# nanoporetech/medaka

Hardware: NVIDIA H100
Metric: pileup positions/sec (consensus inference) (higher is better)
Workload: dtype f32

## Files before the change

### include/medaka_b200.h

```cpp
#ifndef MEDAKA_B200_H
#define MEDAKA_B200_H

#include <stddef.h>
#include <stdint.h>

#ifdef __cplusplus
extern "C" {
#endif

#define MDK_OK 0
#define MDK_ERR_ARG -1
#define MDK_ERR_CUDA -2
#define MDK_ERR_STATE -3
#define MDK_ERR_UNSUPPORTED -4
#define MDK_ERR_NOMEM -5

#define MDK_PREC_TC 0
#define MDK_PREC_FP32 1

#define MDK_REC_AUTO 0
#define MDK_REC_ONE_TILE 1
#define MDK_REC_PINGPONG 2

#define MDK_NORM_TOTAL 0
// ... 184 lines not shown
                            float *ref_q_out, int64_t *n_runs_out, int64_t *n_run_cols_out);

int mdk_variant_columns(int device, const int64_t *minor, const uint8_t *reference,
                        const uint8_t *prediction, uint8_t *out, int64_t len);

int mdk_decode_variants(int device, const float *probs, const int64_t *minor, const uint8_t *ref_code, int64_t n,
                        uint8_t *pred_out, uint8_t *is_var_out, float *pred_q_out, float *ref_q_out, int64_t max_runs,
                        int64_t *run_start, int64_t *run_len, float *run_pred_q, float *run_ref_q,
                        int64_t *n_runs_out);

int mdk_selftest_umma(int device, const float *A, const float *B, float *D, int N, int K,
                      int variant);

int mdk_debug_timeline(mdk_engine *e, int n_last, float *out);
int mdk_debug_read_plog(mdk_engine *e, float *out_host, int64_t n_floats);
int mdk_rl_debug_read(mdk_rl_engine *e, int which, float *out_host, int64_t n_floats);

typedef struct mdk_trainer mdk_trainer;

#define MDK_OPT_RMSPROP 0
#define MDK_OPT_ADAM 1
#define MDK_OPT_NADAM 2
#define MDK_OPT_SGD 3

typedef struct mdk_optim_desc {
    int32_t kind;
    float alpha, beta1, beta2, eps, weight_decay, momentum, dampening, momentum_decay;
    int32_t nesterov;
} mdk_optim_desc;

// ... 49 lines not shown
```

### medaka_b200/csrc/api.cu

```cuda
#include <algorithm>
#include <cstdlib>
#include <cstring>
#include <new>

#include "common.cuh"
#include "gru_pack.cuh"

namespace mdk {

static thread_local std::string g_last_error;

void set_error(const std::string &msg) { g_last_error = msg; }

int cuda_fail(cudaError_t err, const char *what, const char *file, int line) {
    char buf[512];
    snprintf(buf, sizeof(buf), "CUDA error %d (%s) at %s:%d: %s", (int)err, cudaGetErrorString(err), file, line, what);
    g_last_error = buf;
    if (err == cudaErrorMemoryAllocation) {
        cudaGetLastError();
        return MDK_ERR_NOMEM;
    }
    return MDK_ERR_CUDA;
}

// ... 136 lines not shown
}

static int ensure_var(mdk_lane &ln) {
    if (ln.cap_var >= ln.cap_io && ln.d_ref) return MDK_OK;
    dev_free(ln.d_ref); dev_free(ln.d_calls); dev_free(ln.d_pred_q); dev_free(ln.d_ref_q);
    ln.cap_var = 0;
    int rc;
    if ((rc = dev_alloc(&ln.d_ref, (size_t)ln.cap_io))) return rc;
    if ((rc = dev_alloc(&ln.d_calls, (size_t)ln.cap_io))) return rc;
    if ((rc = dev_alloc(&ln.d_pred_q, (size_t)ln.cap_io))) return rc;
    if ((rc = dev_alloc(&ln.d_ref_q, (size_t)ln.cap_io))) return rc;
    ln.cap_var = ln.cap_io;
    return MDK_OK;
}

static int run_forward256(mdk_engine *e, mdk_ws &ws, const float *feats_dev, int64_t B, int64_t T, float *probs_dev,
                          float *logits_dev, uint8_t *labels_dev, uint8_t *quals_dev, const HeadVariant *var) {
    int rc;
    if ((rc = ensure_h1(ws, H2_256))) return rc;
    const int64_t P = B * T;
    cudaStream_t s = ws.stream, s1 = ws.l1_stream;
    const bool tc = e->precision == MDK_PREC_TC;
    const LayerWeights &l0 = e->layer[0], &l1 = e->layer[1];
    float *h0 = static_cast<float *>(ws.h0);
    MDK_CUDA(cudaStreamWaitEvent(s, ws.l1_done, 0));
    MDK_CUDA(cudaEventRecord(e->ev[1], s));
    MDK_CUDA(launch_inproj0(feats_dev, l0.w_in_packed, l0.bias_gi, ws.gi, P, e->desc.num_features,
                            T, tc ? 1 : 0, s, H256));
    MDK_CUDA(cudaEventRecord(e->ev[2], s));
    if (tc) MDK_CUDA(launch_rec256_tc(ws.gi, l0.w_hh_tm, l0.b_hn_tc, h0, B, T, s));
    else MDK_CUDA(launch_rec_fp32(ws.gi, l0.w_hh_t, l0.b_hn, h0, B, T, s, H256));
    MDK_CUDA(cudaEventRecord(e->ev[3], s));
    if (tc) MDK_CUDA(launch_gemm256_tc(h0, l1.w_in_tc, l1.bias_gi_tc, ws.gi, tiled_rows(B, T), s));
    else MDK_CUDA(launch_gemm_fp32(h0, l1.w_in_packed, l1.bias_gi, ws.gi, P, H2_256, GI256_COLS, s));
    MDK_CUDA(cudaEventRecord(e->ev[4], s));
    MDK_CUDA(cudaStreamWaitEvent(s1, e->ev[4], 0));
    if (tc) MDK_CUDA(launch_rec256_tc(ws.gi, l1.w_hh_tm, l1.b_hn_tc, ws.h1, B, T, s1));
    else MDK_CUDA(launch_rec_fp32(ws.gi, l1.w_hh_t, l1.b_hn, ws.h1, B, T, s1, H256));
    MDK_CUDA(cudaEventRecord(e->ev[5], s1));
    MDK_CUDA(cudaEventRecord(ws.l1_done, s1));
    MDK_CUDA(launch_head(ws.h1, e->lin_w, e->lin_b, B, T, tc ? 1 : 0, probs_dev, logits_dev, labels_dev, s1, quals_dev,
                         var, H2_256));
    MDK_CUDA(cudaEventRecord(e->ev[6], s1));
    e->launches += 5;
    e->last.launches = 5;
    ws.last_fused_head = false;
    ws.last_B = B; ws.last_T = T; ws.last_precision = e->precision;
    e->last_ws = (int)(&ws - e->ws);
    return MDK_OK;
}

static int run_forward(mdk_engine *e, mdk_ws &ws, const float *feats_dev, int64_t B, int64_t T, float *probs_dev,
                       float *logits_dev, uint8_t *labels_dev, uint8_t *quals_dev, const HeadVariant *var) {
    int rc;
    if ((rc = prepare_weights(e))) return rc;
    if ((rc = ensure_workspace(e, ws, B, T))) return rc;
    if (e->desc.gru_size == H256)
        return run_forward256(e, ws, feats_dev, B, T, probs_dev, logits_dev, labels_dev, quals_dev, var);
    const int64_t P = B * T;
    cudaStream_t s = ws.stream, s1 = ws.l1_stream;
    const bool tc = e->precision == MDK_PREC_TC;
    int launches = 0;
    const bool fuse_x = tc && e->layer[0].w_x_tm != nullptr;
    const int64_t tiles = (B + WT - 1) / WT;
    const int tiles_per_cta = e->rec_mode == MDK_REC_PINGPONG ? 2
                            : e->rec_mode == MDK_REC_ONE_TILE ? 1
                            : fuse_x || tiles * NDIR > (int64_t)e->sm_count ? 2 : 1;
    const bool fuse_head = tc && !e->keep_act;
    if (!fuse_head && (rc = ensure_h1(ws, H2))) return rc;
    if (!fuse_x) MDK_CUDA(cudaStreamWaitEvent(s, ws.l1_done, 0));
    MDK_CUDA(cudaEventRecord(e->ev[1], s));
    if (!fuse_x) {
        MDK_CUDA(launch_inproj0(feats_dev, e->layer[0].w_in_packed, e->layer[0].bias_gi, ws.gi, P,
                                e->desc.num_features, T, tc ? 1 : 0, s));
        launches++;
    }
    MDK_CUDA(cudaEventRecord(e->ev[2], s));
    if (tc) {
        const RecX fx{feats_dev, e->layer[0].w_x_tm, e->layer[0].bias_gi_tc, e->desc.num_features};
        MDK_CUDA(launch_rec_tc(ws.gi, fuse_x ? &fx : nullptr, e->layer[0].w_hh_tm, e->layer[0].b_hn_tc, tiles_per_cta,
                               OUT_TILES, ws.h0, nullptr, B, T, s));
    } else {
        MDK_CUDA(launch_rec_fp32(ws.gi, e->layer[0].w_hh_t, e->layer[0].b_hn, (float *)ws.h0, B, T, s));
    }
    launches++;
    if (fuse_x) MDK_CUDA(cudaStreamWaitEvent(s, ws.l1_done, 0));
    MDK_CUDA(cudaEventRecord(e->ev[3], s));
    if (tc) MDK_CUDA(launch_gemm_tc(ws.h0, e->layer[1].w_in_tc, e->layer[1].bias_gi_tc, ws.gi, tiled_rows(B, T), e->sm_count, s));
    else MDK_CUDA(launch_gemm_fp32((const float *)ws.h0, e->layer[1].w_in_packed, e->layer[1].bias_gi, ws.gi, P, H2, GI_COLS, s));
    launches++;
    MDK_CUDA(cudaEventRecord(e->ev[4], s));
    MDK_CUDA(cudaStreamWaitEvent(s1, e->ev[4], 0));
    if (tc) {
        MDK_CUDA(launch_rec_tc(ws.gi, nullptr, e->layer[1].w_hh_tm, e->layer[1].b_hn_tc, tiles_per_cta,
                               fuse_head ? OUT_LOGITS : OUT_ROWS, fuse_head ? (void *)ws.plog : ws.h1, e->lin_w, B, T, s1));
    } else {
        MDK_CUDA(launch_rec_fp32(ws.gi, e->layer[1].w_hh_t, e->layer[1].b_hn, ws.h1, B, T, s1));
    }
    launches++;
    MDK_CUDA(cudaEventRecord(e->ev[5], s1));
    MDK_CUDA(cudaEventRecord(ws.l1_done, s1));
    if (fuse_head) MDK_CUDA(launch_head_plog(ws.plog, e->lin_b, B, T, probs_dev, logits_dev, labels_dev, s1, quals_dev, var));
    else MDK_CUDA(launch_head(ws.h1, e->lin_w, e->lin_b, B, T, tc ? 1 : 0, probs_dev, logits_dev, labels_dev, s1, quals_dev,
                              var));
    launches++;
    MDK_CUDA(cudaEventRecord(e->ev[6], s1));
    e->launches += launches;
    e->last.launches = launches;
    ws.last_fused_head = fuse_head;
    ws.last_B = B; ws.last_T = T; ws.last_precision = e->precision;
    e->last_ws = (int)(&ws - e->ws);
    return MDK_OK;
}

static int acquire_lane(mdk_engine *e, int64_t P, int *out) {
    int idx;
    if (P > mdk_engine::SMALL_POS) {
        idx = e->next_big;
        e->next_big = (e->next_big + 1) % mdk_engine::BIG_LANES;
    } else {
        idx = mdk_engine::BIG_LANES + e->next_small;
        e->next_small = (e->next_small + 1) % mdk_engine::SMALL_LANES;
    }
    mdk_lane &ln = e->lane[idx];
    if (ln.busy) {
        MDK_CUDA(cudaEventSynchronize(ln.ev_out));
        ln.busy = false;
    }
    *out = idx;
    return MDK_OK;
}

struct GruCall {
    mdk_engine *e;
    const float *feats = nullptr;
    int64_t B = 0, T = 0;
    const uint8_t *ref = nullptr;

    int open(int64_t windows) {
        const int rc = acquire_lane(e, B * T, &e->open_lane);
        return rc ? rc : ensure_io(e, e->lane[e->open_lane], windows, T);
    }
    int64_t capacity(int64_t len) {
        const mdk_lane &ln = e->lane[e->open_lane];
        return std::min(ln.cap_io / len, ln.cap_feats / (len * e->desc.num_features));
    }
    int stage(int64_t first, int64_t n, int64_t at) {
        const size_t w = (size_t)T * e->desc.num_features;
        mdk_lane &ln = e->lane[e->open_lane];
        MDK_CUDA(cudaMemcpyAsync(ln.d_feats + at * w, feats + first * w, n * w * sizeof(float), cudaMemcpyDefault,
                                 e->copy_in));
        if (ref) {
            int rc;
            if ((rc = ensure_var(ln))) return rc;
            MDK_CUDA(cudaMemcpyAsync(ln.d_ref + at * T, ref + first * T, n * T, cudaMemcpyDefault, e->copy_in));
        }
        return MDK_OK;
    }
    int launch() {
        mdk_lane &ln = e->lane[e->open_lane];
        const Packing &pk = e->pk;
        bool logits = false, labels = false, quals = false, var = false;
        for (const Packing::Piece &p : pk.pieces) {
            logits = logits || p.logits; labels = labels || (p.labels && !p.ref); quals = quals || p.quals;
            var = var || p.ref;
        }
        const HeadVariant hv{ln.d_ref, ln.d_calls, ln.d_pred_q, ln.d_ref_q};
        int rc;
        if (quals && (rc = ensure_quals(ln))) return rc;
        cudaStream_t s = ln.ws->stream;
        e->ev = e->evr[e->fwd_count % mdk_engine::EV_RING];
        e->fwd_count++;
        MDK_CUDA(cudaEventRecord(e->ev[0], s));
        MDK_CUDA(cudaEventRecord(ln.ev_in, e->copy_in));
        MDK_CUDA(cudaStreamWaitEvent(s, ln.ev_in, 0));
        if ((rc = run_forward(e, *ln.ws, ln.d_feats, pk.windows, pk.len, ln.d_probs, logits ? ln.d_logits : nullptr,
                              labels ? ln.d_labels : nullptr, quals ? ln.d_quals : nullptr, var ? &hv : nullptr)))
            return rc;
        MDK_CUDA(cudaEventRecord(e->ev[7], ln.ws->l1_stream));
        if ((rc = copy_back(e->copy_out, pk, ln.ws->l1_stream, ln.d_probs, ln.d_logits, ln.d_labels, ln.d_quals, &hv)))
            return rc;
        MDK_CUDA(cudaEventRecord(ln.ev_out, e->copy_out.stream));
        ln.busy = true;
        return MDK_OK;
    }
};

static int launch_group(mdk_engine *e) { return e->pk.launch(GruCall{e}); }

static int64_t group_limit(mdk_engine *e) {
    return e->group_windows > 0 ? e->group_windows : mdk_engine_preferred_windows(e);
}

static float ev_ms(cudaEvent_t a, cudaEvent_t b) {
    float ms = 0.f;
    if (cudaEventElapsedTime(&ms, a, b) != cudaSuccess) { cudaGetLastError(); return -1.f; }
    return ms;
}

static int check_shapes(const mdk_engine *e, const void *feats, int64_t B, int64_t T, const void *probs) {
    MDK_REQUIRE(e != nullptr, MDK_ERR_ARG, "engine is NULL");
    MDK_REQUIRE(feats != nullptr && probs != nullptr, MDK_ERR_ARG, "forward: feats/probs must not be NULL");
    MDK_REQUIRE(B >= 1 && T >= 1, MDK_ERR_ARG, "forward: need B >= 1 and T >= 1");
// ... 118 lines not shown
    }
    e->stream = e->ws[0].stream;
    for (auto &set : e->evr) for (auto &ev : set) cudaEventCreate(&ev);
    cudaStreamCreateWithFlags(&e->copy_in, cudaStreamNonBlocking);
    for (auto &ev : e->ev_timer) cudaEventCreate(&ev);
    cudaEventCreateWithFlags(&e->ev_join, cudaEventDisableTiming);
    cudaError_t err = create_copy_out(e->copy_out);
    if (err != cudaSuccess) { mdk_engine_destroy(e); return cuda_fail(err, "create_copy_out", __FILE__, __LINE__); }
    *out = e;
    return MDK_OK;
}

int mdk_engine_destroy(mdk_engine *e) {
    if (!e) return MDK_OK;
    cudaSetDevice(e->device);
    for (auto &ws : e->ws) {
        if (ws.stream) cudaStreamSynchronize(ws.stream);
        if (ws.l1_stream) cudaStreamSynchronize(ws.l1_stream);
    }
    destroy_copy_out(e->copy_out);
    for (auto &ws : e->ws) {
        dev_free(ws.gi); dev_free(ws.h1); dev_free(ws.plog);
        if (ws.h0) cudaFree(ws.h0);
        if (ws.stream) cudaStreamDestroy(ws.stream);
        if (ws.l1_stream) cudaStreamDestroy(ws.l1_stream);
        if (ws.l1_done) cudaEventDestroy(ws.l1_done);
    }
    for (auto &ln : e->lane) {
        dev_free(ln.d_feats); dev_free(ln.d_probs); dev_free(ln.d_logits); dev_free(ln.d_labels); dev_free(ln.d_quals);
        dev_free(ln.d_ref); dev_free(ln.d_calls); dev_free(ln.d_pred_q); dev_free(ln.d_ref_q);
        if (ln.ev_in) cudaEventDestroy(ln.ev_in);
        if (ln.ev_out) cudaEventDestroy(ln.ev_out);
    }
    if (e->copy_in) cudaStreamDestroy(e->copy_in);
    for (auto &set : e->evr) for (auto &ev : set) if (ev) cudaEventDestroy(ev);
    for (auto &ev : e->ev_timer) if (ev) cudaEventDestroy(ev);
    if (e->ev_join) cudaEventDestroy(e->ev_join);
    delete e;
    cudaGetLastError();
    return MDK_OK;
}

static int quiesce(mdk_engine *e) {
    int rc = launch_group(e);
    if (rc) return rc;
    for (auto &ws : e->ws) MDK_CUDA(ws_sync(ws));
    return MDK_OK;
}

int mdk_engine_load_gru(mdk_engine *e, int layer, int direction, const float *w_ih, const float *w_hh,
                        const float *b_ih, const float *b_hh) {
    MDK_REQUIRE(e, MDK_ERR_ARG, "engine is NULL");
    MDK_REQUIRE(layer >= 0 && layer < 2 && direction >= 0 && direction < 2, MDK_ERR_ARG, "load_gru: bad layer/direction");
    MDK_REQUIRE(w_ih && w_hh && b_ih && b_hh, MDK_ERR_ARG, "load_gru: NULL weight pointer");
    MDK_CUDA(cudaSetDevice(e->device));
    { int rcq = quiesce(e); if (rcq) return rcq; }
    LayerWeights &lw = e->layer[layer];
    const int g3 = 3 * e->desc.gru_size;
    lw.w_ih[direction].assign(w_ih, w_ih + (size_t)g3 * in_features(e, layer));
// ... 34 lines not shown
                "set_rec_mode: at gru_size 256 the recurrence has one kernel; only MDK_REC_AUTO applies");
    e->rec_mode = mode;
    return MDK_OK;
}

int mdk_engine_set_group_windows(mdk_engine *e, int64_t windows) {
    MDK_REQUIRE(e && windows >= 0, MDK_ERR_ARG, "set_group_windows: bad arguments");
    e->group_windows = windows;
    return MDK_OK;
}

int mdk_engine_reserve(mdk_engine *e, int64_t B, int64_t T) {
    MDK_REQUIRE(e && B >= 1 && T >= 1, MDK_ERR_ARG, "reserve: bad arguments");
    MDK_CUDA(cudaSetDevice(e->device));
    int rc;
    if ((rc = launch_group(e))) return rc;
    if (e->desc.gru_size == H256) B = std::min(B, group_limit(e));
    const bool big = B * T > mdk_engine::SMALL_POS;
    const int l0 = big ? 0 : mdk_engine::BIG_LANES, l1 = big ? mdk_engine::BIG_LANES : mdk_engine::N_LANES;
    for (int i = l0; i < l1; ++i) {
        mdk_lane &ln = e->lane[i];
        if (ln.busy) { MDK_CUDA(cudaEventSynchronize(ln.ev_out)); ln.busy = false; }
        if ((rc = ensure_workspace(e, *ln.ws, B, T))) return rc;
        if ((rc = ensure_io(e, ln, B, T))) return rc;
    }
    return MDK_OK;
}

int mdk_engine_forward_dev(mdk_engine *e, const float *feats_dev, int64_t B, int64_t T, float *probs_dev,
                           float *logits_dev, uint8_t *labels_dev) {
    int rc;
// ... 32 lines not shown
    MDK_REQUIRE(e != nullptr, MDK_ERR_ARG, "engine is NULL");
    MDK_REQUIRE(feats && ref_bytes && calls_out && pred_q_out && ref_q_out, MDK_ERR_ARG,
                "submit_variant_decoded: NULL input or output");
    MDK_REQUIRE(B >= 1 && T >= 1, MDK_ERR_ARG, "submit_variant_decoded: need B >= 1 and T >= 1");
    MDK_REQUIRE(B * T < (int64_t)1 << 40, MDK_ERR_ARG, "submit_variant_decoded: B*T too large");
    MDK_REQUIRE(ticket, MDK_ERR_ARG, "submit_variant_decoded: ticket is NULL");
    MDK_CUDA(cudaSetDevice(e->device));
    GruCall call{e, feats, B, T, ref_bytes};
    return e->pk.enqueue(call, B, T, nullptr, nullptr, calls_out, group_limit(e), ticket, nullptr, ref_bytes,
                         pred_q_out, ref_q_out);
}

int mdk_engine_flush(mdk_engine *e) {
    MDK_REQUIRE(e, MDK_ERR_ARG, "engine is NULL");
    MDK_CUDA(cudaSetDevice(e->device));
    return launch_group(e);
}

int mdk_engine_wait(mdk_engine *e, int64_t ticket) {
    MDK_REQUIRE(e, MDK_ERR_ARG, "engine is NULL");
    MDK_REQUIRE(ticket >= 0 && ticket < e->pk.tickets, MDK_ERR_ARG, "wait: unknown ticket");
    MDK_CUDA(cudaSetDevice(e->device));
    return wait_ticket(e->copy_out, e->pk, GruCall{e}, ticket);
}

int mdk_engine_forward(mdk_engine *e, const float *feats_host, int64_t B, int64_t T, float *probs_host,
                       float *logits_host, uint8_t *labels_host) {
    int64_t ticket = -1;
    int rc = mdk_engine_submit(e, feats_host, B, T, probs_host, logits_host, labels_host, &ticket);
    if (rc) return rc;
    return mdk_engine_wait(e, ticket);
}

int mdk_engine_sync(mdk_engine *e) {
    MDK_REQUIRE(e, MDK_ERR_ARG, "engine is NULL");
    MDK_CUDA(cudaSetDevice(e->device));
    int rc = launch_group(e);
    if (rc) return rc;
    MDK_CUDA(cudaStreamSynchronize(e->copy_in));
    for (auto &ws : e->ws) MDK_CUDA(ws_sync(ws));
    MDK_CUDA(cudaStreamSynchronize(e->copy_out.stream));
    for (auto &ln : e->lane) ln.busy = false;
    return MDK_OK;
}

static void stage_times(cudaEvent_t *ev, mdk_timings *t) {
    t->h2d_ms = ev_ms(ev[0], ev[1]);
    t->inproj0_ms = ev_ms(ev[1], ev[2]);
    t->rec0_ms = ev_ms(ev[2], ev[3]);
    t->inproj1_ms = ev_ms(ev[3], ev[4]);
    t->rec1_ms = ev_ms(ev[4], ev[5]);
    t->head_ms = ev_ms(ev[5], ev[6]);
    t->d2h_ms = ev_ms(ev[6], ev[7]);
    t->total_ms = ev_ms(ev[0], ev[7]);
}

int mdk_engine_last_timings(mdk_engine *e, mdk_timings *out) { return mdk_engine_mean_timings(e, 1, out); }

int mdk_engine_mean_timings(mdk_engine *e, int n_last, mdk_timings *out) {
    MDK_REQUIRE(e && out, MDK_ERR_ARG, "NULL argument");
    MDK_REQUIRE(n_last >= 1 && n_last <= mdk_engine::EV_RING, MDK_ERR_ARG, "mean_timings: n_last out of range");
    MDK_CUDA(cudaSetDevice(e->device));
    int rc = launch_group(e);
    if (rc) return rc;
    MDK_REQUIRE(e->fwd_count >= 1, MDK_ERR_STATE, "mean_timings: no forward recorded");
    n_last = (int)std::min<int64_t>(n_last, e->fwd_count);
    for (auto &ws : e->ws) MDK_CUDA(ws_sync(ws));
    mdk_timings acc{};
    for (int i = 0; i < n_last; ++i) {
        mdk_timings t{};
        stage_times(e->evr[(e->fwd_count - 1 - i) % mdk_engine::EV_RING], &t);
        acc.h2d_ms += t.h2d_ms; acc.inproj0_ms += t.inproj0_ms; acc.rec0_ms += t.rec0_ms;
        acc.inproj1_ms += t.inproj1_ms; acc.rec1_ms += t.rec1_ms; acc.head_ms += t.head_ms;
        acc.d2h_ms += t.d2h_ms; acc.total_ms += t.total_ms;
    }
    const float inv = 1.0f / (float)n_last;
    acc.h2d_ms *= inv; acc.inproj0_ms *= inv; acc.rec0_ms *= inv; acc.inproj1_ms *= inv; acc.rec1_ms *= inv;
    acc.head_ms *= inv; acc.d2h_ms *= inv; acc.total_ms *= inv;
    acc.launches = e->last.launches;
    *out = acc;
    return MDK_OK;
}

int mdk_debug_timeline(mdk_engine *e, int n_last, float *out) {
    MDK_REQUIRE(e && out, MDK_ERR_ARG, "NULL argument");
    MDK_CUDA(cudaSetDevice(e->device));
    int rc = launch_group(e);
    if (rc) return rc;
    MDK_REQUIRE(n_last >= 1 && n_last <= mdk_engine::EV_RING && e->fwd_count >= n_last, MDK_ERR_ARG, "timeline: bad n_last");
    for (auto &ws : e->ws) MDK_CUDA(ws_sync(ws));
    for (int i = 0; i < n_last; ++i) {
        cudaEvent_t *ev = e->evr[(e->fwd_count - n_last + i) % mdk_engine::EV_RING];
        for (int k = 0; k < 8; ++k) MDK_CUDA(cudaEventElapsedTime(out + i * 8 + k, e->ev_timer[0], ev[k]));
    }
    return MDK_OK;
}

int mdk_engine_timer_start(mdk_engine *e) {
    MDK_REQUIRE(e, MDK_ERR_ARG, "engine is NULL");
    MDK_CUDA(cudaSetDevice(e->device));
    int rc = mdk_engine_sync(e);
    if (rc) return rc;
    MDK_CUDA(cudaEventRecord(e->ev_timer[0], e->stream));
    for (int i = 0; i < mdk_engine::N_WS; ++i) {
        if (i) MDK_CUDA(cudaStreamWaitEvent(e->ws[i].stream, e->ev_timer[0], 0));
        MDK_CUDA(cudaStreamWaitEvent(e->ws[i].l1_stream, e->ev_timer[0], 0));
    }
    MDK_CUDA(cudaStreamWaitEvent(e->copy_in, e->ev_timer[0], 0));
    return MDK_OK;
}
int mdk_engine_timer_stop(mdk_engine *e, float *elapsed_ms) {
    MDK_REQUIRE(e && elapsed_ms, MDK_ERR_ARG, "NULL argument");
    MDK_CUDA(cudaSetDevice(e->device));
    int rc = launch_group(e);
    if (rc) return rc;
    for (int i = 0; i < mdk_engine::N_WS; ++i) {
        if (i) {
            MDK_CUDA(cudaEventRecord(e->ev_join, e->ws[i].stream));
            MDK_CUDA(cudaStreamWaitEvent(e->stream, e->ev_join, 0));
        }
        MDK_CUDA(cudaEventRecord(e->ev_join, e->ws[i].l1_stream));
        MDK_CUDA(cudaStreamWaitEvent(e->stream, e->ev_join, 0));
    }
    MDK_CUDA(cudaEventRecord(e->ev_join, e->copy_out.stream));
    MDK_CUDA(cudaStreamWaitEvent(e->stream, e->ev_join, 0));
    MDK_CUDA(cudaEventRecord(e->ev_timer[1], e->stream));
    MDK_CUDA(cudaEventSynchronize(e->ev_timer[1]));
    MDK_CUDA(cudaEventElapsedTime(elapsed_ms, e->ev_timer[0], e->ev_timer[1]));
    return MDK_OK;
// ... 6 lines not shown

int mdk_engine_read_activation_windows(mdk_engine *e, int which, int64_t first, int64_t count, float *out_host,
                                       int64_t n_floats) {
    MDK_REQUIRE(e && out_host, MDK_ERR_ARG, "NULL argument");
    MDK_REQUIRE(which == 0 || which == 1, MDK_ERR_ARG, "read_activation: which must be 0 or 1");
    mdk_ws &ln = e->ws[e->last_ws];
    MDK_REQUIRE(ln.last_B > 0 && ln.last_T > 0, MDK_ERR_STATE, "read_activation: no forward recorded");
    MDK_REQUIRE(first >= 0 && count > 0 && first + count <= ln.last_B, MDK_ERR_ARG,
                "read_activation: windows first .. first + count - 1 must lie in the last forward's B windows");
    const int width = 2 * e->desc.gru_size;
    MDK_REQUIRE(n_floats == count * ln.last_T * width, MDK_ERR_ARG, "read_activation: size must be count*T*2*gru_size");
    MDK_REQUIRE(!(which == 1 && ln.last_fused_head), MDK_ERR_STATE,
                "read_activation(1): the last forward fused the head into layer 1 (h1 never reached HBM); call "
                "mdk_engine_keep_activations(e, 1) before the forward");
    MDK_CUDA(cudaSetDevice(e->device));
    MDK_CUDA(ws_sync(ln));
    if (ln.last_precision == MDK_PREC_FP32) {
        const float *src = (which == 1 ? ln.h1 : reinterpret_cast<const float *>(ln.h0)) + first * ln.last_T * width;
        MDK_CUDA(cudaMemcpy(out_host, src, (size_t)n_floats * sizeof(float), cudaMemcpyDeviceToHost));
    } else {
        float *tmp = nullptr;
        MDK_CUDA(cudaMalloc(&tmp, (size_t)n_floats * sizeof(float)));
        const float *rows = which == 1 ? ln.h1 : static_cast<const float *>(ln.h0);
        cudaError_t err = which == 0 && width == H2 ? launch_unpack_h0(ln.h0, tmp, first, count, ln.last_T, ln.stream)
                                                    : launch_untile_rows(rows, tmp, first, count, ln.last_T, ln.stream, width);
        if (err == cudaSuccess) err = cudaStreamSynchronize(ln.stream);
        if (err == cudaSuccess) err = cudaMemcpy(out_host, tmp, (size_t)n_floats * sizeof(float), cudaMemcpyDeviceToHost);
        cudaFree(tmp);
        e->launches++;
        if (err != cudaSuccess) return cuda_fail(err, "read_activation", __FILE__, __LINE__);
    }
    return MDK_OK;
}


int mdk_debug_read_plog(mdk_engine *e, float *out_host, int64_t n_floats) {
    MDK_REQUIRE(e && out_host, MDK_ERR_ARG, "NULL argument");
    mdk_ws &ln = e->ws[e->last_ws];
    MDK_REQUIRE(ln.last_fused_head, MDK_ERR_STATE, "read_plog: the last forward did not run the fused head");
    const int64_t tiles = (ln.last_B + WT - 1) / WT;
    MDK_REQUIRE(n_floats == NDIR * tiles * ln.last_T * PLOG_TS_FLOATS, MDK_ERR_ARG, "read_plog: size must be 2*tiles*T*80");
    MDK_CUDA(cudaSetDevice(e->device));
    MDK_CUDA(ws_sync(ln));
    MDK_CUDA(cudaMemcpy(out_host, ln.plog, (size_t)n_floats * sizeof(float), cudaMemcpyDeviceToHost));
    return MDK_OK;
}

int64_t mdk_engine_launch_count(mdk_engine *e) { return e ? e->launches : 0; }

int mdk_engine_keep_activations(mdk_engine *e, int keep) {
    MDK_REQUIRE(e, MDK_ERR_ARG, "NULL engine");
    e->keep_act = keep != 0;
    return MDK_OK;
}

int64_t mdk_engine_preferred_windows(mdk_engine *e) {
    if (e && e->desc.gru_size == H256) return e->wave256;
    const int sms = e ? e->sm_count : 132;
    return (int64_t)mdk::WT * (sms / mdk::NDIR);
// ... 10 lines not shown
```

### medaka_b200/csrc/common.cuh

```cuda
#pragma once
#include <cuda_runtime.h>
#include <cuda_fp16.h>

#include <cstdint>
#include <cstdio>
#include <string>
#include <vector>

#include "../../include/medaka_b200.h"
#include "packing.h"

namespace mdk {

constexpr int H = 128;
constexpr int G3 = 3 * H;
constexpr int NDIR = 2;
constexpr int GI_COLS = NDIR * G3;
constexpr int H2 = NDIR * H;
constexpr int NCLS = 5;
constexpr int H256 = 256;
constexpr int G3_256 = 3 * H256;
constexpr int GI256_COLS = NDIR * G3_256;
constexpr int H2_256 = NDIR * H256;

// ... 224 lines not shown
    cudaEvent_t evr[EV_RING][8] = {};
    cudaEvent_t *ev = evr[0];
    int64_t fwd_count = 0;
    cudaEvent_t ev_timer[2] = {};
    cudaEvent_t ev_join = nullptr;
    mdk::LayerWeights layer[2];
    std::vector<float> lin_w_host, lin_b_host;
    float *lin_w = nullptr, *lin_b = nullptr;
    mdk::DeviceWeights weights;
    bool keep_act = false;
    bool prepared = false;
    cudaStream_t copy_in = nullptr;
    mdk::CopyOut copy_out;
    mdk_timings last{};
    int64_t launches = 0;
};

namespace mdk {

cudaError_t launch_inproj0(const float *feats, const float *w_packed, const float *bias, float *gi,
                           int64_t P, int F, int64_t T, int tiled, cudaStream_t s, int hs = H);
enum { HEAD_PLAIN = 0, HEAD_QUALS = 1, HEAD_VARIANT = 2 };
cudaError_t launch_head(const float *h1, const float *lin_w, const float *lin_b, int64_t B, int64_t T, int tiled,
                        float *probs, float *logits, uint8_t *labels, cudaStream_t s, uint8_t *quals = nullptr,
                        const HeadVariant *var = nullptr, int width = H2);
cudaError_t launch_untile_rows(const float *src_tiled, float *dst, int64_t w0, int64_t nw, int64_t T, cudaStream_t s,
                               int width = H2);
cudaError_t launch_unpack_h0(const void *h0_tiles, float *out, int64_t w0, int64_t nw, int64_t T, cudaStream_t s);
cudaError_t launch_rec_fp32(const float *gi, const float *w_hh_t, const float *b_hn, float *h_out, int64_t B,
                            int64_t T, cudaStream_t s, int hs = H, float *save = nullptr);
cudaError_t launch_gemm_fp32(const float *A, const float *W, const float *bias, float *C, int64_t M, int K, int N,
                             cudaStream_t s);
struct RecX {
    const float *feats;
    const __half *w_x;
    const float *bias;
    int F;
};
enum { OUT_TILES = 0, OUT_ROWS = 1, OUT_LOGITS = 2 };
cudaError_t launch_rec_tc(const float *gi, const RecX *xin, const __half *w_hh_tm, const float *b_hn, int tiles_per_cta,
                          int out_kind, void *out, const float *lin_w, int64_t B, int64_t T, cudaStream_t s);
cudaError_t launch_head_plog(const float *plog, const float *lin_b, int64_t B, int64_t T, float *probs, float *logits,
                             uint8_t *labels, cudaStream_t s, uint8_t *quals = nullptr,
                             const HeadVariant *var = nullptr);
constexpr int PLOG_TS_FLOATS = NCLS * WT;
cudaError_t launch_gemm_tc(const void *x_tiles, const __half *w_in_tm, const float *bias, float *gi, int64_t P,
                           int sm_count, cudaStream_t s);
int selftest_umma(int device, const float *A, const float *B, float *D, int N, int K, int variant);
cudaError_t launch_rec256_tc(const float *gi, const __half *w_hh_tm, const float *b_hn, float *h_out, int64_t B,
                             int64_t T, cudaStream_t s);
cudaError_t rec256_max_clusters(int *clusters);
cudaError_t launch_gemm256_tc(const float *h0, const __half *w_in_tm, const float *bias, float *gi, int64_t M,
                              cudaStream_t s);
cudaError_t launch_scan_blocks(int64_t *counts, int64_t n, cudaStream_t s);
struct Records {
// ... 14 lines not shown
```

### medaka_b200/csrc/gru_wg.cu

```cuda
#include "common.cuh"
#include "ptx.cuh"
#include "rec_common.cuh"

namespace mdk {

constexpr int RW_THREADS = 256;
constexpr int RW_ABLK = (H / 8) * 64 * 16;
constexpr int RW_XBLK = 2 * 64 * 16;

template <int NT, bool FUSE_X, int OUT>
struct RwCfg {
    static constexpr int N = NT * RT_N;
    static constexpr bool HL = NT == 1;
    static constexpr int ROWS = HL ? 2 * N : N;
    static constexpr int PLANES = HL ? 1 : 2;
    static constexpr int KG = ROWS * 16 + 16;
    static_assert(KG % 16 == 0, "stmatrix rows are 16-byte aligned");
    static constexpr int HPLANE = (H / 8) * KG;
    static constexpr int XPLANE = 2 * KG;
    static constexpr int HLO = HL ? N * 16 : HPLANE;
    static constexpr int XLO = HL ? N * 16 : XPLANE;
    static constexpr int RED = (RW_THREADS / 32) * NCLS * N;
    static constexpr int wlo_off = 0;
    static constexpr int wxlo_off = wlo_off + 6 * RW_ABLK;
    static constexpr int h_off = wxlo_off + (FUSE_X ? 6 * RW_XBLK : 0);
    static constexpr int x_off = h_off + 2 * PLANES * HPLANE;
    static constexpr int red_off = x_off + (FUSE_X ? 2 * PLANES * XPLANE : 0);
    static constexpr int total = red_off + (OUT == OUT_LOGITS ? 2 * RED * 4 : 0);
    static_assert(total <= 227 * 1024, "smem budget");
};

__device__ __forceinline__ uint32_t ld_u32(const __half *p) { return *reinterpret_cast<const uint32_t *>(p); }

template <int NT, bool FUSE_X, int OUT>
__global__ void __launch_bounds__(RW_THREADS, 1)
rec_tc_kernel(const float *__restrict__ gi, RecX xin, const __half *__restrict__ w_hh, const float *__restrict__ b_hn,
              void *__restrict__ h_out, int64_t B, int64_t T, const float *__restrict__ lin_w,
              float *__restrict__ plog) {
    using L = RwCfg<NT, FUSE_X, OUT>;
    constexpr int N = L::N, NA = N / 2;
    constexpr int NACC = L::ROWS / 2;
    constexpr int NX = FUSE_X ? NACC : NA;
    using MMA = Wgmma<N>;
    using MMA_H = Wgmma<L::ROWS>;
    constexpr bool LOGITS = OUT == OUT_LOGITS;
    extern __shared__ __align__(128) uint8_t smem[];
    const int tid = threadIdx.x, wg = tid >> 7, warp = (tid >> 5) & 3, lane = tid & 31;
    const int gq = lane >> 2, cq = lane & 3;
    const int dir = blockIdx.y;
    const int64_t ntiles = (B + RT_N - 1) / RT_N;
    const int64_t wtile0 = (int64_t)blockIdx.x * NT;
    const int j0 = wg * 64 + warp * 16 + gq;
    const uint32_t sbase = smem_u32(smem);

// ... 290 lines not shown
            }
        }
        if (FUSE_X || step + 1 < T) load_pre(dir ? t - 1 : t + 1);
        fence_proxy_async_smem();
        __syncthreads();
    }
    if (OUT == OUT_TILES) store_h0((int)(T & 1), dir ? 0 : T - 1);
    if (LOGITS) {
        if (T > 1) head_store((int)((T - 1) & 1), dir ? 1 : T - 2);
        head_partials((int)(T & 1));
        __syncthreads();
        head_store((int)(T & 1), dir ? 0 : T - 1);
    }
}

template <int NT, bool FX, int OUT>
static cudaError_t launch_rec(const float *gi, const RecX &xin, const __half *w_hh_tm, const float *b_hn, void *out,
                              const float *lin_w, int64_t B, int64_t T, cudaStream_t s) {
    auto kern = rec_tc_kernel<NT, FX, OUT>;
    constexpr int smem_bytes = RwCfg<NT, FX, OUT>::total;
    cudaError_t e = cudaFuncSetAttribute(kern, cudaFuncAttributeMaxDynamicSharedMemorySize, smem_bytes);
    if (e != cudaSuccess) return e;
    const int64_t tiles = (B + RT_N - 1) / RT_N;
    dim3 grid((unsigned)((tiles + NT - 1) / NT), NDIR);
    constexpr bool LOGITS = OUT == OUT_LOGITS;
    kern<<<grid, RW_THREADS, smem_bytes, s>>>(gi, xin, w_hh_tm, b_hn, LOGITS ? nullptr : out, B, T, lin_w,
                                              LOGITS ? static_cast<float *>(out) : nullptr);
    return cudaGetLastError();
}

template <int NT>
static cudaError_t launch_rec_nt(const float *gi, const RecX *xin, const __half *w_hh_tm, const float *b_hn, int out_kind,
                                 void *out, const float *lin_w, int64_t B, int64_t T, cudaStream_t s) {
    if (xin)
        return out_kind == OUT_TILES ? launch_rec<NT, true, OUT_TILES>(gi, *xin, w_hh_tm, b_hn, out, nullptr, B, T, s)
                                     : cudaErrorInvalidValue;
    const RecX none{nullptr, nullptr, nullptr, 0};
    switch (out_kind) {
    case OUT_TILES: return launch_rec<NT, false, OUT_TILES>(gi, none, w_hh_tm, b_hn, out, nullptr, B, T, s);
    case OUT_ROWS: return launch_rec<NT, false, OUT_ROWS>(gi, none, w_hh_tm, b_hn, out, nullptr, B, T, s);
    case OUT_LOGITS:
        return lin_w ? launch_rec<NT, false, OUT_LOGITS>(gi, none, w_hh_tm, b_hn, out, lin_w, B, T, s) : cudaErrorInvalidValue;
    }
    return cudaErrorInvalidValue;
}

cudaError_t launch_rec_tc(const float *gi, const RecX *xin, const __half *w_hh_tm, const float *b_hn, int tiles_per_cta,
                          int out_kind, void *out, const float *lin_w, int64_t B, int64_t T, cudaStream_t s) {
    if (B == 0 || T == 0) return cudaSuccess;
    switch (tiles_per_cta) {
    case 1: return launch_rec_nt<1>(gi, xin, w_hh_tm, b_hn, out_kind, out, lin_w, B, T, s);
    case 2: return launch_rec_nt<2>(gi, xin, w_hh_tm, b_hn, out_kind, out, lin_w, B, T, s);
    }
    return cudaErrorInvalidValue;
}

constexpr int GW_THREADS = 256;
constexpr int GW_QK = 8;
constexpr int GW_STAGE_PLANE = GW_QK * XT_ROWS * 16;
constexpr int GW_STAGE = 2 * GW_STAGE_PLANE;
constexpr int GW_NQ = XT_K / 8 / GW_QK;
constexpr int GW_KS = XT_K / 16;
constexpr int GW_TS = XT_ROWS / WT;
constexpr int GW_QUAD = H * 4;
constexpr int GW_QUAD_PAD = GW_QUAD + 16;
constexpr int GW_OUT_OFF = GW_NQ * GW_STAGE;
constexpr int GW_BAR_OFF = GW_OUT_OFF + GW_TS * 4 * GW_QUAD_PAD * 4;
// ... 187 lines not shown
```

Baseline: 186.7 million.

## Defer layer-1 recurrence launch and pick recurrence kernel variant by overlap state

Splits the forward pass so the layer-1 recurrence, head and copy-back are issued in a separate step, run_layer1. With fused-x input they are held as pending until the next group opens or a drain occurs. Layer-0 recurrence picks a new one-tile-per-CTA non-HL 'twin' variant when the tile count fits the SM count and the previous layer 1 has already finished, otherwise a two-tile kernel. The aim is to let layer 0 of the next batch overlap the previous layer 1 while using wider per-CTA parallelism when the GPU would otherwise be idle. The cost is more complex state and deferred-flush logic, plus a risk of ordering bugs. It also adds a debug query for the chosen tile counts.

```diff
diff --git a/include/medaka_b200.h b/include/medaka_b200.h
--- a/include/medaka_b200.h
+++ b/include/medaka_b200.h
@@ -222,6 +222,7 @@
 
 int mdk_debug_timeline(mdk_engine *e, int n_last, float *out);
 int mdk_debug_read_plog(mdk_engine *e, float *out_host, int64_t n_floats);
+int mdk_debug_rec_tiles(mdk_engine *e, int n_last, int *out);
 int mdk_rl_debug_read(mdk_rl_engine *e, int which, float *out_host, int64_t n_floats);
 
 typedef struct mdk_trainer mdk_trainer;
diff --git a/medaka_b200/csrc/api.cu b/medaka_b200/csrc/api.cu
--- a/medaka_b200/csrc/api.cu
+++ b/medaka_b200/csrc/api.cu
@@ -174,12 +174,11 @@
     return MDK_OK;
 }
 
-static int run_forward256(mdk_engine *e, mdk_ws &ws, const float *feats_dev, int64_t B, int64_t T, float *probs_dev,
-                          float *logits_dev, uint8_t *labels_dev, uint8_t *quals_dev, const HeadVariant *var) {
+static int run_forward256(mdk_engine *e, mdk_ws &ws, const float *feats_dev, int64_t B, int64_t T) {
     int rc;
     if ((rc = ensure_h1(ws, H2_256))) return rc;
     const int64_t P = B * T;
-    cudaStream_t s = ws.stream, s1 = ws.l1_stream;
+    cudaStream_t s = ws.stream;
     const bool tc = e->precision == MDK_PREC_TC;
     const LayerWeights &l0 = e->layer[0], &l1 = e->layer[1];
     float *h0 = static_cast<float *>(ws.h0);
@@ -194,38 +193,45 @@
     if (tc) MDK_CUDA(launch_gemm256_tc(h0, l1.w_in_tc, l1.bias_gi_tc, ws.gi, tiled_rows(B, T), s));
     else MDK_CUDA(launch_gemm_fp32(h0, l1.w_in_packed, l1.bias_gi, ws.gi, P, H2_256, GI256_COLS, s));
     MDK_CUDA(cudaEventRecord(e->ev[4], s));
-    MDK_CUDA(cudaStreamWaitEvent(s1, e->ev[4], 0));
-    if (tc) MDK_CUDA(launch_rec256_tc(ws.gi, l1.w_hh_tm, l1.b_hn_tc, ws.h1, B, T, s1));
-    else MDK_CUDA(launch_rec_fp32(ws.gi, l1.w_hh_t, l1.b_hn, ws.h1, B, T, s1, H256));
-    MDK_CUDA(cudaEventRecord(e->ev[5], s1));
-    MDK_CUDA(cudaEventRecord(ws.l1_done, s1));
-    MDK_CUDA(launch_head(ws.h1, e->lin_w, e->lin_b, B, T, tc ? 1 : 0, probs_dev, logits_dev, labels_dev, s1, quals_dev,
-                         var, H2_256));
-    MDK_CUDA(cudaEventRecord(e->ev[6], s1));
-    e->launches += 5;
-    e->last.launches = 5;
+    e->launches += 3;
+    e->l1.tc = tc;
+    e->l1.fuse_head = false;
+    e->l1.launches = 3;
+    e->rec_tiles[e->l1.slot][0] = 0;
     ws.last_fused_head = false;
     ws.last_B = B; ws.last_T = T; ws.last_precision = e->precision;
     e->last_ws = (int)(&ws - e->ws);
     return MDK_OK;
 }
 
-static int run_forward(mdk_engine *e, mdk_ws &ws, const float *feats_dev, int64_t B, int64_t T, float *probs_dev,
-                       float *logits_dev, uint8_t *labels_dev, uint8_t *quals_dev, const HeadVariant *var) {
-    int rc;
+static int run_forward(mdk_engine *e, mdk_ws &ws, const float *feats_dev, int *l1_kernel) {
+    int rc;
+    const int64_t B = e->l1.B, T = e->l1.T;
+    *l1_kernel = REC_NT2;
     if ((rc = prepare_weights(e))) return rc;
     if ((rc = ensure_workspace(e, ws, B, T))) return rc;
-    if (e->desc.gru_size == H256)
-        return run_forward256(e, ws, feats_dev, B, T, probs_dev, logits_dev, labels_dev, quals_dev, var);
+    if (e->desc.gru_size == H256) return run_forward256(e, ws, feats_dev, B, T);
     const int64_t P = B * T;
-    cudaStream_t s = ws.stream, s1 = ws.l1_stream;
+    cudaStream_t s = ws.stream;
     const bool tc = e->precision == MDK_PREC_TC;
     int launches = 0;
     const bool fuse_x = tc && e->layer[0].w_x_tm != nullptr;
     const int64_t tiles = (B + WT - 1) / WT;
-    const int tiles_per_cta = e->rec_mode == MDK_REC_PINGPONG ? 2
-                            : e->rec_mode == MDK_REC_ONE_TILE ? 1
-                            : fuse_x || tiles * NDIR > (int64_t)e->sm_count ? 2 : 1;
+    const bool fits = tiles * NDIR <= (int64_t)e->sm_count;
+    int k0 = REC_NT2;
+    if (e->rec_mode == MDK_REC_PINGPONG) {
+        k0 = *l1_kernel = REC_NT2;
+    } else if (e->rec_mode == MDK_REC_ONE_TILE) {
+        k0 = *l1_kernel = REC_NT1_HL;
+    } else if (fuse_x) {
+        const cudaError_t q = cudaEventQuery(ws.l1_done);
+        if (q == cudaErrorNotReady) cudaGetLastError();
+        else if (q != cudaSuccess) return cuda_fail(q, "cudaEventQuery(l1_done)", __FILE__, __LINE__);
+        k0 = fits && q == cudaSuccess ? REC_NT1_TWIN : REC_NT2;
+        *l1_kernel = -1;
+    } else {
+        k0 = *l1_kernel = fits ? REC_NT1_HL : REC_NT2;
+    }
     const bool fuse_head = tc && !e->keep_act;
     if (!fuse_head && (rc = ensure_h1(ws, H2))) return rc;
     if (!fuse_x) MDK_CUDA(cudaStreamWaitEvent(s, ws.l1_done, 0));
@@ -238,8 +244,8 @@
     MDK_CUDA(cudaEventRecord(e->ev[2], s));
     if (tc) {
         const RecX fx{feats_dev, e->layer[0].w_x_tm, e->layer[0].bias_gi_tc, e->desc.num_features};
-        MDK_CUDA(launch_rec_tc(ws.gi, fuse_x ? &fx : nullptr, e->layer[0].w_hh_tm, e->layer[0].b_hn_tc, tiles_per_cta,
-                               OUT_TILES, ws.h0, nullptr, B, T, s));
+        MDK_CUDA(launch_rec_tc(ws.gi, fuse_x ? &fx : nullptr, e->layer[0].w_hh_tm, e->layer[0].b_hn_tc, k0, OUT_TILES,
+                               ws.h0, nullptr, B, T, s));
     } else {
         MDK_CUDA(launch_rec_fp32(ws.gi, e->layer[0].w_hh_t, e->layer[0].b_hn, (float *)ws.h0, B, T, s));
     }
@@ -250,27 +256,55 @@
     else MDK_CUDA(launch_gemm_fp32((const float *)ws.h0, e->layer[1].w_in_packed, e->layer[1].bias_gi, ws.gi, P, H2, GI_COLS, s));
     launches++;
     MDK_CUDA(cudaEventRecord(e->ev[4], s));
-    MDK_CUDA(cudaStreamWaitEvent(s1, e->ev[4], 0));
-    if (tc) {
-        MDK_CUDA(launch_rec_tc(ws.gi, nullptr, e->layer[1].w_hh_tm, e->layer[1].b_hn_tc, tiles_per_cta,
-                               fuse_head ? OUT_LOGITS : OUT_ROWS, fuse_head ? (void *)ws.plog : ws.h1, e->lin_w, B, T, s1));
-    } else {
-        MDK_CUDA(launch_rec_fp32(ws.gi, e->layer[1].w_hh_t, e->layer[1].b_hn, ws.h1, B, T, s1));
-    }
-    launches++;
-    MDK_CUDA(cudaEventRecord(e->ev[5], s1));
-    MDK_CUDA(cudaEventRecord(ws.l1_done, s1));
-    if (fuse_head) MDK_CUDA(launch_head_plog(ws.plog, e->lin_b, B, T, probs_dev, logits_dev, labels_dev, s1, quals_dev, var));
-    else MDK_CUDA(launch_head(ws.h1, e->lin_w, e->lin_b, B, T, tc ? 1 : 0, probs_dev, logits_dev, labels_dev, s1, quals_dev,
-                              var));
-    launches++;
-    MDK_CUDA(cudaEventRecord(e->ev[6], s1));
     e->launches += launches;
-    e->last.launches = launches;
+    e->l1.tc = tc;
+    e->l1.fuse_head = fuse_head;
+    e->l1.launches = launches;
+    e->rec_tiles[e->l1.slot][0] = tc ? rec_tiles_per_cta(k0) : 0;
     ws.last_fused_head = fuse_head;
     ws.last_B = B; ws.last_T = T; ws.last_precision = e->precision;
     e->last_ws = (int)(&ws - e->ws);
     return MDK_OK;
+}
+
+static int run_layer1(mdk_engine *e, int kernel) {
+    mdk_engine::Layer1 &p = e->l1;
+    p.pending = false;
+    mdk_lane &ln = e->lane[p.lane];
+    mdk_ws &ws = *ln.ws;
+    cudaStream_t s1 = ws.l1_stream;
+    cudaEvent_t *ev = e->evr[p.slot];
+    const LayerWeights &lw = e->layer[1];
+    const bool wide = e->desc.gru_size == H256;
+    const int64_t B = p.B, T = p.T;
+    const HeadVariant *var = p.var ? &p.hv : nullptr;
+    MDK_CUDA(cudaStreamWaitEvent(s1, ev[4], 0));
+    if (wide && p.tc) MDK_CUDA(launch_rec256_tc(ws.gi, lw.w_hh_tm, lw.b_hn_tc, ws.h1, B, T, s1));
+    else if (p.tc)
+        MDK_CUDA(launch_rec_tc(ws.gi, nullptr, lw.w_hh_tm, lw.b_hn_tc, kernel, p.fuse_head ? OUT_LOGITS : OUT_ROWS,
+                               p.fuse_head ? (void *)ws.plog : ws.h1, e->lin_w, B, T, s1));
+    else MDK_CUDA(launch_rec_fp32(ws.gi, lw.w_hh_t, lw.b_hn, ws.h1, B, T, s1, wide ? H256 : H));
+    MDK_CUDA(cudaEventRecord(ev[5], s1));
+    MDK_CUDA(cudaEventRecord(ws.l1_done, s1));
+    if (p.fuse_head) MDK_CUDA(launch_head_plog(ws.plog, e->lin_b, B, T, p.probs, p.logits, p.labels, s1, p.quals, var));
+    else MDK_CUDA(launch_head(ws.h1, e->lin_w, e->lin_b, B, T, p.tc ? 1 : 0, p.probs, p.logits, p.labels, s1, p.quals,
+                              var, wide ? H2_256 : H2));
+    MDK_CUDA(cudaEventRecord(ev[6], s1));
+    e->launches += 2;
+    e->last.launches = p.launches + 2;
+    e->rec_tiles[p.slot][1] = p.tc && !wide ? rec_tiles_per_cta(kernel) : 0;
+    MDK_CUDA(cudaEventRecord(ev[7], s1));
+    int rc;
+    if ((rc = copy_back(e->copy_out, e->pk, s1, ln.d_probs, ln.d_logits, ln.d_labels, ln.d_quals, &p.hv))) return rc;
+    MDK_CUDA(cudaEventRecord(ln.ev_out, e->copy_out.stream));
+    ln.busy = true;
+    return MDK_OK;
+}
+
+static int flush_layer1(mdk_engine *e, bool drain) {
+    if (!e->l1.pending) return MDK_OK;
+    const int64_t tiles = (e->l1.B + WT - 1) / WT;
+    return run_layer1(e, drain && tiles * NDIR <= (int64_t)e->sm_count ? REC_NT1_TWIN : REC_NT2);
 }
 
 static int acquire_lane(mdk_engine *e, int64_t P, int *out) {
@@ -298,6 +332,8 @@
     const uint8_t *ref = nullptr;
 
     int open(int64_t windows) {
+        int rc0 = flush_layer1(e, false);
+        if (rc0) return rc0;
         const int rc = acquire_lane(e, B * T, &e->open_lane);
         return rc ? rc : ensure_io(e, e->lane[e->open_lane], windows, T);
     }
@@ -325,28 +361,41 @@
             logits = logits || p.logits; labels = labels || (p.labels && !p.ref); quals = quals || p.quals;
             var = var || p.ref;
         }
-        const HeadVariant hv{ln.d_ref, ln.d_calls, ln.d_pred_q, ln.d_ref_q};
         int rc;
         if (quals && (rc = ensure_quals(ln))) return rc;
         cudaStream_t s = ln.ws->stream;
-        e->ev = e->evr[e->fwd_count % mdk_engine::EV_RING];
+        mdk_engine::Layer1 &g = e->l1;
+        g.lane = e->open_lane;
+        g.slot = (int)(e->fwd_count % mdk_engine::EV_RING);
+        g.B = pk.windows;
+        g.T = pk.len;
+        g.probs = ln.d_probs;
+        g.logits = logits ? ln.d_logits : nullptr;
+        g.labels = labels ? ln.d_labels : nullptr;
+        g.quals = quals ? ln.d_quals : nullptr;
+        g.hv = HeadVariant{ln.d_ref, ln.d_calls, ln.d_pred_q, ln.d_ref_q};
+        g.var = var;
+        e->ev = e->evr[g.slot];
         e->fwd_count++;
         MDK_CUDA(cudaEventRecord(e->ev[0], s));
         MDK_CUDA(cudaEventRecord(ln.ev_in, e->copy_in));
         MDK_CUDA(cudaStreamWaitEvent(s, ln.ev_in, 0));
-        if ((rc = run_forward(e, *ln.ws, ln.d_feats, pk.windows, pk.len, ln.d_probs, logits ? ln.d_logits : nullptr,
-                              labels ? ln.d_labels : nullptr, quals ? ln.d_quals : nullptr, var ? &hv : nullptr)))
-            return rc;
-        MDK_CUDA(cudaEventRecord(e->ev[7], ln.ws->l1_stream));
-        if ((rc = copy_back(e->copy_out, pk, ln.ws->l1_stream, ln.d_probs, ln.d_logits, ln.d_labels, ln.d_quals, &hv)))
-            return rc;
-        MDK_CUDA(cudaEventRecord(ln.ev_out, e->copy_out.stream));
-        ln.busy = true;
-        return MDK_OK;
+        int l1_kernel = REC_NT2;
+        if ((rc = run_forward(e, *ln.ws, ln.d_feats, &l1_kernel))) return rc;
+        if (l1_kernel < 0) {
+            g.pending = true;
+            return MDK_OK;
+        }
+        return run_layer1(e, l1_kernel);
     }
 };
 
 static int launch_group(mdk_engine *e) { return e->pk.launch(GruCall{e}); }
+
+static int drain(mdk_engine *e) {
+    const int rc = launch_group(e);
+    return rc ? rc : flush_layer1(e, true);
+}
 
 static int64_t group_limit(mdk_engine *e) {
     return e->group_windows > 0 ? e->group_windows : mdk_engine_preferred_windows(e);
@@ -495,6 +544,7 @@
 int mdk_engine_destroy(mdk_engine *e) {
     if (!e) return MDK_OK;
     cudaSetDevice(e->device);
+    flush_layer1(e, true);
     for (auto &ws : e->ws) {
         if (ws.stream) cudaStreamSynchronize(ws.stream);
         if (ws.l1_stream) cudaStreamSynchronize(ws.l1_stream);
@@ -523,7 +573,7 @@
 }
 
 static int quiesce(mdk_engine *e) {
-    int rc = launch_group(e);
+    int rc = drain(e);
     if (rc) return rc;
     for (auto &ws : e->ws) MDK_CUDA(ws_sync(ws));
     return MDK_OK;
@@ -588,7 +638,7 @@
     MDK_REQUIRE(e && B >= 1 && T >= 1, MDK_ERR_ARG, "reserve: bad arguments");
     MDK_CUDA(cudaSetDevice(e->device));
     int rc;
-    if ((rc = launch_group(e))) return rc;
+    if ((rc = drain(e))) return rc;
     if (e->desc.gru_size == H256) B = std::min(B, group_limit(e));
     const bool big = B * T > mdk_engine::SMALL_POS;
     const int l0 = big ? 0 : mdk_engine::BIG_LANES, l1 = big ? mdk_engine::BIG_LANES : mdk_engine::N_LANES;
@@ -651,14 +701,19 @@
 int mdk_engine_flush(mdk_engine *e) {
     MDK_REQUIRE(e, MDK_ERR_ARG, "engine is NULL");
     MDK_CUDA(cudaSetDevice(e->device));
-    return launch_group(e);
+    return drain(e);
 }
 
 int mdk_engine_wait(mdk_engine *e, int64_t ticket) {
     MDK_REQUIRE(e, MDK_ERR_ARG, "engine is NULL");
     MDK_REQUIRE(ticket >= 0 && ticket < e->pk.tickets, MDK_ERR_ARG, "wait: unknown ticket");
     MDK_CUDA(cudaSetDevice(e->device));
-    return wait_ticket(e->copy_out, e->pk, GruCall{e}, ticket);
+    int64_t g = 0;
+    int rc = e->pk.settle(GruCall{e}, ticket, &g);
+    if (rc) return rc;
+    if (e->l1.pending && g >= e->pk.launched && (rc = flush_layer1(e, !(e->pk.open && e->pk.windows > 0)))) return rc;
+    MDK_CUDA(cudaEventSynchronize(e->copy_out.ev[g % CopyOut::RING]));
+    return MDK_OK;
 }
 
 int mdk_engine_forward(mdk_engine *e, const float *feats_host, int64_t B, int64_t T, float *probs_host,
@@ -672,7 +727,7 @@
 int mdk_engine_sync(mdk_engine *e) {
     MDK_REQUIRE(e, MDK_ERR_ARG, "engine is NULL");
     MDK_CUDA(cudaSetDevice(e->device));
-    int rc = launch_group(e);
+    int rc = drain(e);
     if (rc) return rc;
     MDK_CUDA(cudaStreamSynchronize(e->copy_in));
     for (auto &ws : e->ws) MDK_CUDA(ws_sync(ws));
@@ -698,7 +753,7 @@
     MDK_REQUIRE(e && out, MDK_ERR_ARG, "NULL argument");
     MDK_REQUIRE(n_last >= 1 && n_last <= mdk_engine::EV_RING, MDK_ERR_ARG, "mean_timings: n_last out of range");
     MDK_CUDA(cudaSetDevice(e->device));
-    int rc = launch_group(e);
+    int rc = drain(e);
     if (rc) return rc;
     MDK_REQUIRE(e->fwd_count >= 1, MDK_ERR_STATE, "mean_timings: no forward recorded");
     n_last = (int)std::min<int64_t>(n_last, e->fwd_count);
@@ -722,7 +777,7 @@
 int mdk_debug_timeline(mdk_engine *e, int n_last, float *out) {
     MDK_REQUIRE(e && out, MDK_ERR_ARG, "NULL argument");
     MDK_CUDA(cudaSetDevice(e->device));
-    int rc = launch_group(e);
+    int rc = drain(e);
     if (rc) return rc;
     MDK_REQUIRE(n_last >= 1 && n_last <= mdk_engine::EV_RING && e->fwd_count >= n_last, MDK_ERR_ARG, "timeline: bad n_last");
     for (auto &ws : e->ws) MDK_CUDA(ws_sync(ws));
@@ -749,7 +804,7 @@
 int mdk_engine_timer_stop(mdk_engine *e, float *elapsed_ms) {
     MDK_REQUIRE(e && elapsed_ms, MDK_ERR_ARG, "NULL argument");
     MDK_CUDA(cudaSetDevice(e->device));
-    int rc = launch_group(e);
+    int rc = drain(e);
     if (rc) return rc;
     for (int i = 0; i < mdk_engine::N_WS; ++i) {
         if (i) {
@@ -786,6 +841,8 @@
                 "read_activation(1): the last forward fused the head into layer 1 (h1 never reached HBM); call "
                 "mdk_engine_keep_activations(e, 1) before the forward");
     MDK_CUDA(cudaSetDevice(e->device));
+    int rc = flush_layer1(e, true);
+    if (rc) return rc;
     MDK_CUDA(ws_sync(ln));
     if (ln.last_precision == MDK_PREC_FP32) {
         const float *src = (which == 1 ? ln.h1 : reinterpret_cast<const float *>(ln.h0)) + first * ln.last_T * width;
@@ -813,8 +870,25 @@
     const int64_t tiles = (ln.last_B + WT - 1) / WT;
     MDK_REQUIRE(n_floats == NDIR * tiles * ln.last_T * PLOG_TS_FLOATS, MDK_ERR_ARG, "read_plog: size must be 2*tiles*T*80");
     MDK_CUDA(cudaSetDevice(e->device));
+    int rc = flush_layer1(e, true);
+    if (rc) return rc;
     MDK_CUDA(ws_sync(ln));
     MDK_CUDA(cudaMemcpy(out_host, ln.plog, (size_t)n_floats * sizeof(float), cudaMemcpyDeviceToHost));
+    return MDK_OK;
+}
+
+int mdk_debug_rec_tiles(mdk_engine *e, int n_last, int *out) {
+    MDK_REQUIRE(e && out, MDK_ERR_ARG, "NULL argument");
+    MDK_CUDA(cudaSetDevice(e->device));
+    int rc = drain(e);
+    if (rc) return rc;
+    MDK_REQUIRE(n_last >= 1 && n_last <= mdk_engine::EV_RING && e->fwd_count >= n_last, MDK_ERR_ARG,
+                "rec_tiles: bad n_last");
+    for (int i = 0; i < n_last; ++i) {
+        const int *t = e->rec_tiles[(e->fwd_count - n_last + i) % mdk_engine::EV_RING];
+        out[2 * i] = t[0];
+        out[2 * i + 1] = t[1];
+    }
     return MDK_OK;
 }
 
diff --git a/medaka_b200/csrc/common.cuh b/medaka_b200/csrc/common.cuh
--- a/medaka_b200/csrc/common.cuh
+++ b/medaka_b200/csrc/common.cuh
@@ -262,6 +262,19 @@
     mdk::CopyOut copy_out;
     mdk_timings last{};
     int64_t launches = 0;
+    struct Layer1 {
+        bool pending = false;
+        int lane = 0;
+        int slot = 0;
+        int64_t B = 0, T = 0;
+        bool tc = true, fuse_head = true;
+        float *probs = nullptr, *logits = nullptr;
+        uint8_t *labels = nullptr, *quals = nullptr;
+        mdk::HeadVariant hv{};
+        bool var = false;
+        int launches = 0;
+    } l1;
+    int rec_tiles[EV_RING][2] = {};
 };
 
 namespace mdk {
@@ -286,7 +299,9 @@
     int F;
 };
 enum { OUT_TILES = 0, OUT_ROWS = 1, OUT_LOGITS = 2 };
-cudaError_t launch_rec_tc(const float *gi, const RecX *xin, const __half *w_hh_tm, const float *b_hn, int tiles_per_cta,
+enum { REC_NT1_HL = 1, REC_NT2 = 2, REC_NT1_TWIN = 3 };
+constexpr int rec_tiles_per_cta(int kernel) { return kernel == REC_NT2 ? 2 : 1; }
+cudaError_t launch_rec_tc(const float *gi, const RecX *xin, const __half *w_hh_tm, const float *b_hn, int kernel,
                           int out_kind, void *out, const float *lin_w, int64_t B, int64_t T, cudaStream_t s);
 cudaError_t launch_head_plog(const float *plog, const float *lin_b, int64_t B, int64_t T, float *probs, float *logits,
                              uint8_t *labels, cudaStream_t s, uint8_t *quals = nullptr,
diff --git a/medaka_b200/csrc/gru_wg.cu b/medaka_b200/csrc/gru_wg.cu
--- a/medaka_b200/csrc/gru_wg.cu
+++ b/medaka_b200/csrc/gru_wg.cu
@@ -8,10 +8,11 @@
 constexpr int RW_ABLK = (H / 8) * 64 * 16;
 constexpr int RW_XBLK = 2 * 64 * 16;
 
-template <int NT, bool FUSE_X, int OUT>
+template <int NT, bool FUSE_X, int OUT, bool HL_>
 struct RwCfg {
+    static_assert(NT == 1 || !HL_, "hi and lo share one operand at one tile per CTA only");
     static constexpr int N = NT * RT_N;
-    static constexpr bool HL = NT == 1;
+    static constexpr bool HL = HL_;
     static constexpr int ROWS = HL ? 2 * N : N;
     static constexpr int PLANES = HL ? 1 : 2;
     static constexpr int KG = ROWS * 16 + 16;
@@ -32,12 +33,12 @@
 
 __device__ __forceinline__ uint32_t ld_u32(const __half *p) { return *reinterpret_cast<const uint32_t *>(p); }
 
-template <int NT, bool FUSE_X, int OUT>
+template <int NT, bool FUSE_X, int OUT, bool HL>
 __global__ void __launch_bounds__(RW_THREADS, 1)
 rec_tc_kernel(const float *__restrict__ gi, RecX xin, const __half *__restrict__ w_hh, const float *__restrict__ b_hn,
               void *__restrict__ h_out, int64_t B, int64_t T, const float *__restrict__ lin_w,
               float *__restrict__ plog) {
-    using L = RwCfg<NT, FUSE_X, OUT>;
+    using L = RwCfg<NT, FUSE_X, OUT, HL>;
     constexpr int N = L::N, NA = N / 2;
     constexpr int NACC = L::ROWS / 2;
     constexpr int NX = FUSE_X ? NACC : NA;
@@ -358,11 +359,11 @@
     }
 }
 
-template <int NT, bool FX, int OUT>
+template <int NT, bool HL, bool FX, int OUT>
 static cudaError_t launch_rec(const float *gi, const RecX &xin, const __half *w_hh_tm, const float *b_hn, void *out,
                               const float *lin_w, int64_t B, int64_t T, cudaStream_t s) {
-    auto kern = rec_tc_kernel<NT, FX, OUT>;
-    constexpr int smem_bytes = RwCfg<NT, FX, OUT>::total;
+    auto kern = rec_tc_kernel<NT, FX, OUT, HL>;
+    constexpr int smem_bytes = RwCfg<NT, FX, OUT, HL>::total;
     cudaError_t e = cudaFuncSetAttribute(kern, cudaFuncAttributeMaxDynamicSharedMemorySize, smem_bytes);
     if (e != cudaSuccess) return e;
     const int64_t tiles = (B + RT_N - 1) / RT_N;
@@ -373,28 +374,32 @@
     return cudaGetLastError();
 }
 
-template <int NT>
+template <int NT, bool HL>
 static cudaError_t launch_rec_nt(const float *gi, const RecX *xin, const __half *w_hh_tm, const float *b_hn, int out_kind,
                                  void *out, const float *lin_w, int64_t B, int64_t T, cudaStream_t s) {
     if (xin)
-        return out_kind == OUT_TILES ? launch_rec<NT, true, OUT_TILES>(gi, *xin, w_hh_tm, b_hn, out, nullptr, B, T, s)
+        return out_kind == OUT_TILES ? launch_rec<NT, HL, true, OUT_TILES>(gi, *xin, w_hh_tm, b_hn, out, nullptr, B, T, s)
                                      : cudaErrorInvalidValue;
     const RecX none{nullptr, nullptr, nullptr, 0};
     switch (out_kind) {
-    case OUT_TILES: return launch_rec<NT, false, OUT_TILES>(gi, none, w_hh_tm, b_hn, out, nullptr, B, T, s);
-    case OUT_ROWS: return launch_rec<NT, false, OUT_ROWS>(gi, none, w_hh_tm, b_hn, out, nullptr, B, T, s);
+    case OUT_TILES:
+        if constexpr (HL || NT == 2) return launch_rec<NT, HL, false, OUT_TILES>(gi, none, w_hh_tm, b_hn, out, nullptr, B, T, s);
+        return cudaErrorInvalidValue;
+    case OUT_ROWS: return launch_rec<NT, HL, false, OUT_ROWS>(gi, none, w_hh_tm, b_hn, out, nullptr, B, T, s);
     case OUT_LOGITS:
-        return lin_w ? launch_rec<NT, false, OUT_LOGITS>(gi, none, w_hh_tm, b_hn, out, lin_w, B, T, s) : cudaErrorInvalidValue;
+        return lin_w ? launch_rec<NT, HL, false, OUT_LOGITS>(gi, none, w_hh_tm, b_hn, out, lin_w, B, T, s)
+                     : cudaErrorInvalidValue;
     }
     return cudaErrorInvalidValue;
 }
 
-cudaError_t launch_rec_tc(const float *gi, const RecX *xin, const __half *w_hh_tm, const float *b_hn, int tiles_per_cta,
+cudaError_t launch_rec_tc(const float *gi, const RecX *xin, const __half *w_hh_tm, const float *b_hn, int kernel,
                           int out_kind, void *out, const float *lin_w, int64_t B, int64_t T, cudaStream_t s) {
     if (B == 0 || T == 0) return cudaSuccess;
-    switch (tiles_per_cta) {
-    case 1: return launch_rec_nt<1>(gi, xin, w_hh_tm, b_hn, out_kind, out, lin_w, B, T, s);
-    case 2: return launch_rec_nt<2>(gi, xin, w_hh_tm, b_hn, out_kind, out, lin_w, B, T, s);
+    switch (kernel) {
+    case REC_NT1_HL: return launch_rec_nt<1, true>(gi, xin, w_hh_tm, b_hn, out_kind, out, lin_w, B, T, s);
+    case REC_NT2: return launch_rec_nt<2, false>(gi, xin, w_hh_tm, b_hn, out_kind, out, lin_w, B, T, s);
+    case REC_NT1_TWIN: return launch_rec_nt<1, false>(gi, xin, w_hh_tm, b_hn, out_kind, out, lin_w, B, T, s);
     }
     return cudaErrorInvalidValue;
 }
```

Result: faster. 190.1 million (median of 6 runs) (+1.8%).
